# smritip/real-time-audio-sync

Measured on AMD Instinct MI355X. Metric: aligned chroma frames/sec, batch=64 OTW c=500; path-index match vs CPU ref, higher is better.
Workload: dtype f64 arithmetic, f32 features in HBM

## Files before the change

### real_time_audio_sync_amd/csrc/otw.hip

```cpp
#include <hip/hip_runtime.h>
#include <math.h>
#include <stddef.h>
#include <stdint.h>
#include <stdlib.h>
#include <string.h>
#include <type_traits>

#include "common.h"

namespace rts {

constexpr int kF = 12;
constexpr int kFetch = 8;

struct OtwArgs {
    const void *ref;
    const void *live;
    const int32_t *live_len;
    int32_t *state;
    int32_t *path;
    double *bands;
    long long live_stride;
    int N, c, max_run_count, variant, cost_kind, mode;
    int path_cap, live_cap;
    int ref_f64, live_f64;
    int clamp_len;
    long long *debug;
    int spec;
    double *dense_acc;
    double *dense_cost;
    const long long *ref_first;
    const int32_t *ref_len;
};

struct LiveFromGlobal {};
struct LiveFromGlobalLean {};
template <typename RT> struct RingElem { using type = RT; };
template <> struct RingElem<LiveFromGlobal> { using type = float; };
template <> struct RingElem<LiveFromGlobalLean> { using type = float; };
template <typename RT> constexpr bool kThroughput = std::is_same<RT, LiveFromGlobalLean>::value;
template <typename RT> constexpr bool kHasLiveRing = !std::is_same<RT, LiveFromGlobal>::value && !kThroughput<RT>;

template <int W, typename RT>
struct OtwLds {
    static constexpr int L = W / 64;
    static constexpr int SWZ = L * 65;
    double R[SWZ];
    double C[SWZ];
    double Dr[2][SWZ];
    double Dc[2][SWZ];
    using E = typename RingElem<RT>::type;
    E livew[kF][kHasLiveRing<RT> ? W : 1];
    double cfresh_min;
    double corner_pa;
    double corner_d;
    int cfresh_idx;
    int rfresh_idx;
    double rfresh_min;
    int plan_t[2], plan_j0[2], plan_flags[2];
    int t, j;
    E refw[kF][W];
};

struct OtwSpecOut {
    double min;
    double d;
    double d2;
    int idx;
    int flag;
};
template <int W>
struct alignas(16) OtwSpecLds {
    static constexpr int SWZ = (W / 64) * 65;
    double ShR[SWZ];
    double ShC[SWZ];
    OtwSpecOut row[2], col[2];
};

template <int W>
__device__ __forceinline__ int swz(int k) {
    constexpr int L = W / 64;
    const int p = k & (W - 1);
    return (p % L) * 65 + (p / L);
}

__device__ __forceinline__ double dmin(double a, double b) { return (b < a) ? b : a; }

__device__ __forceinline__ double dot_strided12(const double (&x)[kF], const double (&y)[kF]) {
    double t1 = 0.0, t2 = 0.0;
#pragma unroll
    for (int i = 0; i < kF; i += 4) {
        const double m3 = y[i + 2] * x[i + 2];
        const double m4 = y[i + 3] * x[i + 3];
        const double a = fma(y[i], x[i], m3);
        const double b = fma(y[i + 1], x[i + 1], m4);
        t1 = t1 + a;
        t2 = t2 + b;
    }
    return t1 + t2;
}

__device__ __forceinline__ double euclid12(const double (&a)[kF], const double (&b)[kF]) {
    double sq[kF];
#pragma unroll
    for (int i = 0; i < kF; i++) {
        const double d = a[i] - b[i];
        sq[i] = d * d;
    }
    double res = ((sq[0] + sq[1]) + (sq[2] + sq[3])) + ((sq[4] + sq[5]) + (sq[6] + sq[7]));
    res = res + sq[8];
    res = res + sq[9];
    res = res + sq[10];
    res = res + sq[11];
    return sqrt(res);
}

__device__ __forceinline__ double cell_cost(const double (&lf)[kF], const double (&rf)[kF], int euclid) {
    return euclid ? euclid12(lf, rf) : (1.0 - dot_strided12(lf, rf));
}

__device__ __forceinline__ double vmin(double a, double b) {
    double r;
    asm("v_min_f64 %0, %1, %2" : "=v"(r) : "v"(a), "v"(b));
    return r;
}

__device__ __forceinline__ double wave_shift_up(double v, double lane0) {
    const int lo = __builtin_amdgcn_update_dpp(__double2loint(lane0), __double2loint(v), 0x138, 0xf, 0xf, false);
    const int hi = __builtin_amdgcn_update_dpp(__double2hiint(lane0), __double2hiint(v), 0x138, 0xf, 0xf, false);
    return __hiloint2double(hi, lo);
}

__device__ __forceinline__ double wave_bcast(double v, int src_lane) {
    const int lo = __builtin_amdgcn_readlane(__double2loint(v), src_lane);
    const int hi = __builtin_amdgcn_readlane(__double2hiint(v), src_lane);
    return __hiloint2double(hi, lo);
}

__device__ __forceinline__ double rfl(double v) {
    const int lo = __builtin_amdgcn_readfirstlane(__double2loint(v));
    const int hi = __builtin_amdgcn_readfirstlane(__double2hiint(v));
    return __hiloint2double(hi, lo);
}

#define RTS_DPP_MIN_STEP(CTRL, ROWMASK)                                                                       \
    do {                                                                                                      \
        const int tlo = __builtin_amdgcn_update_dpp(__double2loint(x), __double2loint(x), CTRL, ROWMASK, 0xf, false); \
        const int thi = __builtin_amdgcn_update_dpp(__double2hiint(x), __double2hiint(x), CTRL, ROWMASK, 0xf, false); \
        x = vmin(x, __hiloint2double(thi, tlo));                                                              \
    } while (0)

__device__ __forceinline__ double wave_min(double x) {
    RTS_DPP_MIN_STEP(0x111, 0xf);
    RTS_DPP_MIN_STEP(0x112, 0xf);
    RTS_DPP_MIN_STEP(0x114, 0xf);
    RTS_DPP_MIN_STEP(0x118, 0xf);
    RTS_DPP_MIN_STEP(0x142, 0xa);
    RTS_DPP_MIN_STEP(0x143, 0xc);
    return wave_bcast(x, 63);
}

__device__ __forceinline__ unsigned lds_addr(const double *p) {
    return (unsigned)(uintptr_t)(__attribute__((address_space(3))) const double *)p;
}
template <int OFF>
__device__ __forceinline__ double lds_read_imm(unsigned addr) {
    double r;
    asm volatile("ds_read_b64 %0, %1 offset:%2" : "=v"(r) : "v"(addr), "n"(OFF));
    return r;
}
template <int OFF>
__device__ __forceinline__ void lds_write_imm(unsigned addr, double v) {
    asm volatile("ds_write_b64 %0, %1 offset:%2" ::"v"(addr), "v"(v), "n"(OFF) : "memory");
}
template <int L, int R, int M = 0>
__device__ __forceinline__ void chain_load(unsigned bA, unsigned bB, unsigned dA, unsigned dB, double (&prevb)[L + 1],
                                           double (&D)[L]) {
    if constexpr (M <= L) {
        constexpr int off = ((R + M) & (L - 1)) * 65 * 8;
        constexpr bool wrap = (R + M) >= L;
        prevb[M] = lds_read_imm<off>(wrap ? bB : bA);
        if constexpr (M > 0) D[M - 1] = lds_read_imm<off>(wrap ? dB : dA);
        chain_load<L, R, M + 1>(bA, bB, dA, dB, prevb, D);
    }
}
template <int L, int M = 0>
__device__ __forceinline__ void chain_wait(double (&prevb)[L + 1], double (&D)[L]) {
    if constexpr (M == 0) asm volatile("s_waitcnt lgkmcnt(0)" ::: "memory");
    if constexpr (M <= L) {
        asm volatile("" : "+v"(prevb[M]));
        if constexpr (M < L) asm volatile("" : "+v"(D[M]));
        chain_wait<L, M + 1>(prevb, D);
    }
}
template <int L, int R, int M = 1>
__device__ __forceinline__ void chain_store(unsigned oA, unsigned oB, const double (&v)[L], double v_top) {
    if constexpr (M <= L) {
        constexpr int off = ((R + M) & (L - 1)) * 65 * 8;
        lds_write_imm<off>((R + M) >= L ? oB : oA, (M == L) ? v_top : v[M - 1]);
        chain_store<L, R, M + 1>(oA, oB, v, v_top);
    }
}

template <int W, bool DENSE, bool GUARD = false, bool ALT = false>
__device__ __forceinline__ void strip_chain(const double *__restrict__ Dv, const double *band, double *band_out, int k1,
                                            int n, double x_in, int lane, int lo_arg, double &fmin_out, int &fidx_out,
                                            double *dense_acc, double *dense_cost, long long dense_stride,
                                            long long *rounds_acc = nullptr, bool prev0_xin = false, double alt_xin = 0.0,
                                            int *alt_ok = nullptr) {
    constexpr int L = W / 64;
    constexpr int LOG_L = (L == 1) ? 0 : (L == 2) ? 1 : (L == 4) ? 2 : (L == 8) ? 3 : (L == 16) ? 4 : 5;
    const double inf = INFINITY;
    int slot[L + 1];
    const int nloc = n - L * lane;
    double prevb[L + 1], D[L], v[L];
    const int q0 = k1 - 1 + W;
    const int r0 = q0 & (L - 1);
    const int colA = ((q0 >> LOG_L) + lane) & 63, colB = (colA + 1) & 63;
    if constexpr (GUARD) {
        const unsigned bA = lds_addr(band + colA), bB = lds_addr(band + colB), dA = lds_addr(Dv + colA), dB = lds_addr(Dv + colB);
        switch (r0) {
#define RTS_CHAIN_LOAD(R)                                                        \
    case R:                                                                      \
        if constexpr (R < L) chain_load<L, R>(bA, bB, dA, dB, prevb, D);         \
        break;
            RTS_CHAIN_LOAD(0) RTS_CHAIN_LOAD(1) RTS_CHAIN_LOAD(2) RTS_CHAIN_LOAD(3) RTS_CHAIN_LOAD(4) RTS_CHAIN_LOAD(5)
            RTS_CHAIN_LOAD(6) RTS_CHAIN_LOAD(7) RTS_CHAIN_LOAD(8) RTS_CHAIN_LOAD(9) RTS_CHAIN_LOAD(10) RTS_CHAIN_LOAD(11)
            RTS_CHAIN_LOAD(12) RTS_CHAIN_LOAD(13) RTS_CHAIN_LOAD(14) RTS_CHAIN_LOAD(15)
            RTS_CHAIN_LOAD(16) RTS_CHAIN_LOAD(17) RTS_CHAIN_LOAD(18) RTS_CHAIN_LOAD(19) RTS_CHAIN_LOAD(20) RTS_CHAIN_LOAD(21)
            RTS_CHAIN_LOAD(22) RTS_CHAIN_LOAD(23) RTS_CHAIN_LOAD(24) RTS_CHAIN_LOAD(25) RTS_CHAIN_LOAD(26) RTS_CHAIN_LOAD(27)
            RTS_CHAIN_LOAD(28) RTS_CHAIN_LOAD(29) RTS_CHAIN_LOAD(30) RTS_CHAIN_LOAD(31)
#undef RTS_CHAIN_LOAD
        }
        chain_wait<L>(prevb, D);
    } else {
#pragma unroll
        for (int m = 0; m <= L; m++) {
            const int q = k1 + m - 1 + W;
            slot[m] = (q & (L - 1)) * 65 + (((q >> LOG_L) + lane) & 63);
        }
#pragma unroll
        for (int m = 0; m <= L; m++) prevb[m] = band[slot[m]];
#pragma unroll
        for (int m = 0; m < L; m++) D[m] = Dv[slot[m + 1]];
    }
    prevb[0] = (k1 == 0 && lane == 0) ? inf : prevb[0];
    if (GUARD && ALT) prevb[0] = (prev0_xin && lane == 0) ? x_in : prevb[0];
#pragma unroll
    for (int m = 0; m < L; m++) D[m] = (m < nloc) ? D[m] : inf;
    double p = (lane == 0) ? x_in : inf;
    double am1 = inf;
#pragma unroll
    for (int m = 0; m < L; m++) {
        const double am = vmin(prevb[m + 1] + D[m], prevb[m] + 2 * D[m]);
        if (GUARD && ALT && m == 1) am1 = am;
        p = p + D[m];
        v[m] = vmin(am, p);
        p = v[m];
    }
    if (GUARD && ALT && L >= 2) {
        if (alt_ok) *alt_ok = __builtin_amdgcn_readfirstlane((int)(vmin(am1, alt_xin + D[1]) == v[1]));
    }
    for (int round = 0; round < 64; round++) {
        double q = wave_shift_up(v[L - 1], x_in);
        q = q + D[0];
        if (!__any(q < v[0])) break;
        if (rounds_acc) *rounds_acc += 1;
        v[0] = vmin(v[0], q);
#pragma unroll
        for (int m = 1; m < L; m++) {
            q = q + D[m];
            v[m] = vmin(v[m], q);
        }
    }
    if constexpr (GUARD) {
        const double v_top = (lane == 63) ? x_in : v[L - 1];
        const unsigned oA = lds_addr(band_out + colA), oB = lds_addr(band_out + colB);
        switch (r0) {
#define RTS_CHAIN_STORE(R)                                                       \
    case R:                                                                      \
        if constexpr (R < L) chain_store<L, R>(oA, oB, v, v_top);                \
        break;
            RTS_CHAIN_STORE(0) RTS_CHAIN_STORE(1) RTS_CHAIN_STORE(2) RTS_CHAIN_STORE(3) RTS_CHAIN_STORE(4)
            RTS_CHAIN_STORE(5) RTS_CHAIN_STORE(6) RTS_CHAIN_STORE(7) RTS_CHAIN_STORE(8) RTS_CHAIN_STORE(9)
            RTS_CHAIN_STORE(10) RTS_CHAIN_STORE(11) RTS_CHAIN_STORE(12) RTS_CHAIN_STORE(13) RTS_CHAIN_STORE(14)
            RTS_CHAIN_STORE(15) RTS_CHAIN_STORE(16) RTS_CHAIN_STORE(17) RTS_CHAIN_STORE(18) RTS_CHAIN_STORE(19)
            RTS_CHAIN_STORE(20) RTS_CHAIN_STORE(21) RTS_CHAIN_STORE(22) RTS_CHAIN_STORE(23) RTS_CHAIN_STORE(24)
            RTS_CHAIN_STORE(25) RTS_CHAIN_STORE(26) RTS_CHAIN_STORE(27) RTS_CHAIN_STORE(28) RTS_CHAIN_STORE(29)
            RTS_CHAIN_STORE(30) RTS_CHAIN_STORE(31)
#undef RTS_CHAIN_STORE
        }
    } else {
#pragma unroll
        for (int m = 0; m < L; m++) band_out[slot[m + 1]] = v[m];
    }
    if (DENSE) {
#pragma unroll
        for (int m = 0; m < L; m++) {
            if (m < nloc) {
                const long long off = (long long)(L * lane + m) * dense_stride;
                dense_acc[off] = v[m];
                dense_cost[off] = D[m];
            }
        }
    }
    const double v0 = (lane == 0 && lo_arg > k1) ? inf : v[0];
    double lm = v0;
#pragma unroll
    for (int m = 1; m < L; m++) lm = vmin(lm, v[m]);
    const double g = wave_min(lm);
    int ml = L;
#pragma unroll
    for (int m = L - 1; m >= 1; m--) ml = (v[m] == g) ? m : ml;
    ml = (v0 == g) ? 0 : ml;
    const unsigned long long mask = __ballot(ml != L);
    const bool some = (g < inf) && (mask != 0);
    const int first = (int)__builtin_ctzll(mask | (1ull << 63));
    fmin_out = g;
    fidx_out = some ? k1 + L * first + __builtin_amdgcn_readlane(ml, first) : 0x7fffffff;
}

template <int W>
__device__ __forceinline__ void band_argmin(const double *__restrict__ band, int lo, int hi, int lane,
                                            double &vmin_out, int &imin) {
    constexpr int L = W / 64;
    double v[L];
    double lm = INFINITY;
#pragma unroll
    for (int m = 0; m < L; m++) {
        const int k = lo + L * lane + m;
        v[m] = (k <= hi) ? band[swz<W>(k)] : (double)INFINITY;
        if (k <= hi) lm = vmin(lm, v[m]);
    }
    const double g = wave_min(lm);
    int cand = 0x7fffffff;
#pragma unroll
    for (int m = L - 1; m >= 0; m--) {
        const int k = lo + L * lane + m;
        if (k <= hi && v[m] == g) cand = k;
    }
    const unsigned long long mask = __ballot(cand != 0x7fffffff);
    vmin_out = g;
    imin = mask ? __builtin_amdgcn_readlane(cand, (int)__builtin_ctzll(mask)) : 0x7fffffff;
}

#if defined(RTS_OTW_STAMPS) && RTS_OTW_STAMPS == 1
#define RTS_STAMP2(slot)      \
    do {                      \
        if (stamp_base)       \
            RTS_STAMP(8 + slot); \
        else                  \
            RTS_STAMP(slot);  \
    } while (0)
#define RTS_STAMP(slot)                                                   \
    do {                                                                  \
        const long long now_ = (long long)__builtin_amdgcn_s_memtime();   \
        __builtin_amdgcn_s_waitcnt(0xC07F);                               \
        stamp_sum[slot] += now_ - stamp_last;                             \
        stamp_last = now_;                                                \
    } while (0)
#else
#define RTS_STAMP(slot) \
    do {                \
    } while (0)
#define RTS_STAMP2(slot) \
    do {                 \
    } while (0)
#endif

struct OtwCtl {
    int t, j, dir, prev, run_count, status, first, n_path, consumed, rows, cols, truncated, pend_dir;
    int recomputes, pending_col, last_x, last_y, rb_idx, cb_idx;
    int live_hi, ref_hi;
    int spec_valid;
    int ri, ci;
    double cA, cU, cL;
    long long cells;
    double rb_min, cb_min;
    double pfl0, pfl1, pfr0, pfr1;
};

struct OtwEnv {
    int b, lane, c, N, live_len, live_cap, euclid, variant, mode, max_run_count, path_cap, live_f64, ref_f64;
    long long live_base;
    const void *live, *ref;
    int32_t *path;
    bool deferred_update;
};

constexpr int kPlanRow = 1, kPlanCol = 2, kPlanStop = 4, kPlanExit = 8;
constexpr int kPlanHit = 16;
constexpr int kPlanRi = 32, kPlanCi = 64;
// ... 466 lines not shown
        otw_ref_frame(e, kb_c, rb);
        const double da = cell_cost(lf, ra, e.euclid), db = cell_cost(lf, rb, e.euclid);
        Drow[swz<W>(ka)] = da;
        if (ka >= dual_lo) S.Dc[ka & 1][swz<W>(r)] = da;
        if (kb <= k_hi) {
            Drow[swz<W>(kb)] = db;
            if (kb >= dual_lo) S.Dc[kb & 1][swz<W>(r)] = db;
        }
    }
}
template <int W, typename RT>
__device__ __forceinline__ void otw_cost_col(OtwLds<W, RT> &S, const OtwEnv &e, int q, int r_lo, int r_hi, int dual_lo,
                                             int hidx, int hn) {
    if (q >= e.N) return;
    const int lim = (e.live_len < e.live_cap) ? e.live_len : e.live_cap;
    if (r_lo < 0) r_lo = 0;
    if (r_hi > lim - 1) r_hi = lim - 1;
    if (r_lo + hidx > r_hi) return;
    double *Dcol = S.Dc[q & 1];
    double rf[kF];
    otw_ref_frame(e, q, rf);
    if constexpr (kThroughput<RT>) {
        for (int ra_ = r_lo + hidx; ra_ <= r_hi; ra_ += hn) {
            double la[kF];
            otw_live_frame(e, ra_, la);
            const double da = cell_cost(la, rf, e.euclid);
            Dcol[swz<W>(ra_)] = da;
            if (ra_ >= dual_lo) S.Dr[ra_ & 1][swz<W>(q)] = da;
        }
        return;
    }
    for (int ra_ = r_lo + hidx; ra_ <= r_hi; ra_ += 2 * hn) {
        const int rb_ = ra_ + hn;
        const int rb_c = (rb_ <= r_hi) ? rb_ : ra_;
        double la[kF], lb[kF];
        if constexpr (!kHasLiveRing<RT>) {
            otw_live_frame(e, ra_, la);
            otw_live_frame(e, rb_c, lb);
        } else {
#pragma unroll
            for (int f = 0; f < kF; f++) {
                la[f] = (double)S.livew[f][ra_ & (W - 1)];
                lb[f] = (double)S.livew[f][rb_c & (W - 1)];
            }
        }
        const double da = cell_cost(la, rf, e.euclid), db = cell_cost(lb, rf, e.euclid);
        Dcol[swz<W>(ra_)] = da;
        if (ra_ >= dual_lo) S.Dr[ra_ & 1][swz<W>(q)] = da;
        if (rb_ <= r_hi) {
            Dcol[swz<W>(rb_)] = db;
            if (rb_ >= dual_lo) S.Dr[rb_ & 1][swz<W>(q)] = db;
        }
    }
}

template <int W, typename RT>
__device__ __forceinline__ void otw_costs_prime(OtwLds<W, RT> &S, const OtwEnv &e, int t, int j, int hidx, int hn) {
    const int c = e.c;
    const int none = 0x7fffffff;
    otw_cost_row<W, RT>(S, e, t + 1, j - c + 1, j + 2, none, hidx, hn);
    otw_cost_row<W, RT>(S, e, t + 2, j - c + 1, j + 2, none, hidx, hn);
    otw_cost_col<W, RT>(S, e, j + 1, t - c + 1, t + 2, none, hidx, hn);
    otw_cost_col<W, RT>(S, e, j + 2, t - c + 1, t + 2, none, hidx, hn);
}

template <int W, typename RT>
__device__ __forceinline__ void otw_costs_advance(OtwLds<W, RT> &S, const OtwEnv &e, int pt, int jn, bool do_row,
                                                  bool do_col, int hidx, int hn) {
    const int c = e.c;
    if (do_row) otw_cost_row<W, RT>(S, e, pt + 2, jn - c + 1, jn + 2, jn + 1, hidx, hn);
    if (do_col) otw_cost_col<W, RT>(S, e, jn + 2, pt - c + 1, pt + 2, pt + 1, hidx, hn);
}

template <int W, bool ALT>
__device__ __forceinline__ void otw_spec_strip(const double *Dv, const double *band, double *shadow, int pos, int c,
                                               int lane, double sentinel, OtwSpecOut *out, long long *rounds_acc = nullptr,
                                               bool prev0_sentinel = false) {
    const int k1 = (pos - c + 1 > 0) ? pos - c + 1 : 0;
    double fm;
    int fi;
    const double d_last = Dv[swz<W>(pos)];
    const double d_next = Dv[swz<W>(pos + 1)];
    int alt_ok = 0;
    strip_chain<W, false, true, ALT>(Dv, band, shadow, k1, pos - k1, (k1 > 0) ? sentinel : (double)INFINITY, lane, k1, fm, fi,
                                nullptr, nullptr, 0, rounds_acc, prev0_sentinel, sentinel, &alt_ok);
    if (lane == 0) {
        out->min = fm;
        out->idx = fi;
        out->d = d_last;
        out->d2 = d_next;
        out->flag = alt_ok;
    }
}

__device__ __forceinline__ double otw_last_cell_from(double prev_raw, int pos, int k1, double side_v, double diag_v, double d,
                                                     double sentinel) {
    const double inf = INFINITY;
    const int n = pos - k1;
    const double prev = (n > 0) ? prev_raw : ((k1 > 0) ? sentinel : inf);
    const double diag = (pos > 0) ? diag_v + 2 * d : inf;
    return vmin(vmin(side_v + d, diag), prev + d);
}
template <int W>
__device__ __forceinline__ double otw_last_cell(const double *band, int pos, int k1, double side_v, double diag_v, double d,
                                                double sentinel) {
    const int n = pos - k1;
    return otw_last_cell_from(band[swz<W>(pos - (n > 0 ? 1 : 0))], pos, k1, side_v, diag_v, d, sentinel);
}

template <int W, typename RT>
__device__ __forceinline__ OtwSettled otw_settle_hit_both(double *R, double *C, const OtwSpecOut *exr, const OtwSpecOut *exc,
                                                          OtwCtl &k, const OtwEnv &e, int pt, int j0, double sentinel) {
    const int c = e.c, lane = e.lane;
    const int jn = j0 + 1, t0 = pt - 1;
    if (e.deferred_update && k.pend_dir != -2) {
        k.run_count = (k.pend_dir == k.prev) ? k.run_count + 1 : 1;
        if (k.pend_dir != RTS_DIR_BOTH) k.prev = k.pend_dir;
        k.pend_dir = -2;
    }
    const int k1r_ = (j0 - c + 1 > 0) ? j0 - c + 1 : 0, k1c_ = (pt - c + 1 > 0) ? pt - c + 1 : 0;
    const double pra_raw = R[swz<W>(j0 - (j0 - k1r_ > 0 ? 1 : 0))], prb_raw = C[swz<W>(t0 - (t0 - k1c_ > 0 ? 1 : 0))];
    const double d1_raw = exr->d, d2_raw = exc->d, d3_raw = exc->d2, rmin_raw = exr->min, cmin_raw = exc->min;
    const int ridx_raw = exr->idx, cidx_raw = exc->idx;
    const double d1 = rfl(d1_raw), d2 = rfl(d2_raw), d3 = rfl(d3_raw);
    double rmin = rfl(rmin_raw), cmin = rfl(cmin_raw);
    int ridx = __builtin_amdgcn_readfirstlane(ridx_raw), cidx = __builtin_amdgcn_readfirstlane(cidx_raw);
    const double pra = rfl(pra_raw), prb = rfl(prb_raw);
    const int k1r = (j0 - c + 1 > 0) ? j0 - c + 1 : 0, k1c = (pt - c + 1 > 0) ? pt - c + 1 : 0;
    const int lo_r = (jn - c + 1 > 0) ? jn - c + 1 : 0;
    const int k1c_s = (t0 - c + 1 > 0) ? t0 - c + 1 : 0;
    const double a = rfl(otw_last_cell_from(pra, j0, k1r, k.cA, k.cL, d1, sentinel));
    const double b = rfl(otw_last_cell_from(prb, t0, k1c, k.cA, k.cU, d2, sentinel));
    const double pa = k.cA + 2 * d3;
    const double av = vmin(a + d3, pa);
    const double cl = vmin(av, b + d3);
    if (lane == 0) {
        R[swz<W>(j0)] = a;
        C[swz<W>(t0)] = b;
        R[swz<W>(jn)] = cl;
        C[swz<W>(pt)] = cl;
        if (k1c > k1c_s) C[swz<W>(k1c - 1)] = sentinel;
    }
    if (a < rmin) {
        rmin = a;
        ridx = j0;
    }
    if (b < cmin) {
        cmin = b;
        cidx = t0;
    }
    const bool row_ok = ridx >= lo_r, col_ok = cidx >= k1c;
    if (!row_ok) k.rb_idx = -1;
    if (!col_ok) k.cb_idx = -1;
    k.rows += 1;
    k.cols += 1;
    k.consumed = pt + 1;
    k.cells += (j0 - k1r + 1) + (pt - k1c + 1);
    k.cU = b;
    k.cL = a;
    k.cA = cl;
    OtwSettled o;
    o.row_fresh = row_ok;
    o.col_fresh = col_ok;
    o.rf_min = rmin;
    o.rf_idx = ridx;
    o.cf_min = cmin;
    o.cf_idx = cidx;
    o.row_corner = o.col_corner = true;
    o.rc = o.cc = cl;
    o.stop = false;
    return o;
}

__device__ __forceinline__ int otw_resolve_plan(int pflags, int pt, int c, const OtwSpecOut *exc) {
    if (pflags & kPlanHitIf) {
        const bool ok = (pt < c) || __builtin_amdgcn_readfirstlane(exc->flag) != 0;
        if (ok) pflags = (pflags | kPlanHit) ^ (kPlanRi | kPlanCi);
    }
    return pflags;
}

template <int W, typename RT>
__device__ __forceinline__ OtwSettled otw_settle_hit(double *R, double *C, const OtwSpecOut *ex, OtwCtl &k, const OtwEnv &e,
                                                     int pt, int j0, bool is_row, double sentinel) {
    const int c = e.c, lane = e.lane;
    const double inf = INFINITY;
    const int jn = j0 + (is_row ? 0 : 1);
    const int pos = is_row ? j0 : pt;
    const int k1 = (pos - c + 1 > 0) ? pos - c + 1 : 0;
    const int n = pos - k1;
    double *band = is_row ? R : C;
    double *other = is_row ? C : R;
    if (e.deferred_update && k.pend_dir != -2) {
        k.run_count = (k.pend_dir == k.prev) ? k.run_count + 1 : 1;
        if (k.pend_dir != RTS_DIR_BOTH) k.prev = k.pend_dir;
        k.pend_dir = -2;
    }
    const double prev_raw = band[swz<W>(pos - (n > 0 ? 1 : 0))];
    const double d_raw = ex->d, smin_raw = ex->min;
    const int sidx_raw = ex->idx;
    const double d = rfl(d_raw);
    const double smin = rfl(smin_raw);
    const int sidx = __builtin_amdgcn_readfirstlane(sidx_raw);
    const double prev_s = rfl(prev_raw);
    const double prev = (n > 0) ? prev_s : ((k1 > 0) ? sentinel : inf);
    const double side = k.cA + d;
    const double diag = (pos > 0) ? (is_row ? k.cL : k.cU) + 2 * d : inf;
    const double cl = vmin(vmin(side, diag), prev + d);
    if (lane == 0) {
        band[swz<W>(pos)] = cl;
        other[swz<W>(is_row ? pt : jn)] = cl;
    }
    if (is_row) {
        k.rows += 1;
        k.consumed = pt + 1;
        k.cU = k.cA;
        k.cL = prev;
    } else {
        k.cols += 1;
        k.cL = k.cA;
        k.cU = prev;
    }
    k.cA = cl;
    k.cells += n + 1;
    OtwSettled o;
    o.row_fresh = is_row;
    o.col_fresh = !is_row;
    o.rf_min = o.cf_min = smin;
    o.rf_idx = o.cf_idx = sidx;
    o.row_corner = o.col_corner = true;
    o.rc = o.cc = cl;
    o.stop = false;
    return o;
}

#ifdef RTS_OTW_FULL_BARRIER
#define RTS_STEP_BARRIER() __syncthreads()
#else
#define RTS_STEP_BARRIER() ::rts::lds_barrier()
#endif

template <int W, int NW, bool DENSE, typename RT, bool SPEC>
__global__ void __launch_bounds__(64 * NW) __attribute__((amdgpu_waves_per_eu(kThroughput<RT> ? 6 : 1)))
otw_advance_kernel(OtwArgs a) {
    static_assert(!SPEC || (NW >= 8 && !DENSE), "the pipelined kernel needs 8 waves and no dense mirror");
    constexpr int NT = 64 * NW;
    constexpr int HW0 = SPEC ? 3 : (NW >= 4) ? 2 : 0;
    constexpr int NHELP = 64 * (NW - HW0);
#if defined(RTS_OTW_STAMPS) && RTS_OTW_STAMPS == 1
    long long stamp_sum[16] = {0, 0, 0, 0, 0, 0, 0, 0, 0, 0, 0, 0, 0, 0, 0, 0};
    int stamp_base = 0;
    long long stamp_last = (long long)__builtin_amdgcn_s_memtime();
    __builtin_amdgcn_s_waitcnt(0xC07F);
#endif
#if defined(RTS_OTW_STAMPS) && RTS_OTW_STAMPS == 2
    long long lw_hit = 0, lb_hit = 0, lw_oth = 0, lb_oth = 0, ln_hit = 0, ln_oth = 0, l_last = 0;
    long long lo_work = 0, lo_t0 = 0;
    long long lo_rounds = 0;
#define RTS_ROUNDS_ACC (&lo_rounds)
#define RTS_LW_BEGIN() do { lo_t0 = (long long)__builtin_amdgcn_s_memtime(); __builtin_amdgcn_s_waitcnt(0xC07F); } while (0)
#define RTS_LW_END(hit) do { const long long t_ = (long long)__builtin_amdgcn_s_memtime(); __builtin_amdgcn_s_waitcnt(0xC07F); if (hit) lo_work += t_ - lo_t0; } while (0)
#else
#define RTS_ROUNDS_ACC nullptr
#define RTS_LW_BEGIN() do { } while (0)
#define RTS_LW_END(hit) do { } while (0)
#endif
    extern __shared__ __align__(16) unsigned char smem_raw[];
    OtwLds<W, RT> &S = *reinterpret_cast<OtwLds<W, RT> *>(smem_raw);
    using LdsT = OtwLds<W, RT>;
    constexpr bool kNoLiveRing = !kHasLiveRing<RT>;
    constexpr bool kRefRing = !SPEC && !kNoLiveRing;
    constexpr size_t kSpecOff = (offsetof(LdsT, refw) + 15) & ~(size_t)15;
    OtwSpecLds<W> &SP = *reinterpret_cast<OtwSpecLds<W> *>(smem_raw + kSpecOff);

    const int tid = threadIdx.x;
    const int lane = tid & 63;
    const int wave = __builtin_amdgcn_readfirstlane(tid >> 6);
    const double sentinel = (a.variant == RTS_VARIANT_OTW) ? 1e10 : (double)INFINITY;
    const double inf = INFINITY;
    OtwEnv e;
    e.b = blockIdx.x;
    e.lane = lane;
    e.c = a.c;
    e.euclid = a.cost_kind == RTS_COST_EUCLID;
    e.variant = a.variant;
    e.mode = a.mode;
// ... 189 lines not shown
                const int pt = __builtin_amdgcn_readfirstlane(S.plan_t[sp]), j0 = __builtin_amdgcn_readfirstlane(S.plan_j0[sp]);
                const int pflags = otw_resolve_plan(__builtin_amdgcn_readfirstlane(S.plan_flags[sp]), pt, c, &SP.col[sp]);
                if (pflags & kPlanExit) break;
                const bool do_row = (pflags & kPlanRow) != 0, do_col = (pflags & kPlanCol) != 0;
                RTS_LW_BEGIN();
                if constexpr (!kNoLiveRing)
                    if (wave == HW0) otw_refill<W, RT>(S, k, e, pt + 3, 0, false);
                if (!(pflags & kPlanHit)) RTS_STEP_BARRIER();
                if (!(pflags & kPlanStop))
                    otw_costs_advance<W, RT>(S, e, pt, j0 + (do_col ? 1 : 0), do_row, do_col, tid - 64 * HW0, NHELP);
                RTS_LW_END(pflags & kPlanHit);
                RTS_STEP_BARRIER();
                sp ^= 1;
            }
        } else if (wave == 1) {
            for (;;) {
                const int pt = __builtin_amdgcn_readfirstlane(S.plan_t[sp]), j0 = __builtin_amdgcn_readfirstlane(S.plan_j0[sp]);
                const int pflags = otw_resolve_plan(__builtin_amdgcn_readfirstlane(S.plan_flags[sp]), pt, c, &SP.col[sp]);
                if (pflags & kPlanExit) break;
                const int jn = j0 + ((pflags & kPlanCol) ? 1 : 0);
                double *R = (pflags & kPlanRi) ? SP.ShR : S.R, *Rsh = (pflags & kPlanRi) ? S.R : SP.ShR;
                RTS_LW_BEGIN();
                if (!(pflags & kPlanHit)) {
                    if ((pflags & (kPlanRow | kPlanCol | kPlanStop)) == (kPlanRow | kPlanCol))
                        otw_col_strip<W, DENSE, RT>(S, (pflags & kPlanCi) ? SP.ShC : S.C, a, e, S.Dc[(j0 + 1) & 1], pt,
                                                    j0 + 1, true, sentinel);
                    RTS_STEP_BARRIER();
                }
                if ((pflags & (kPlanHit | kPlanRow | kPlanCol)) == (kPlanHit | kPlanRow | kPlanCol)) {
                    const double av = otw_last_cell<W>(R, j0, (j0 - c + 1 > 0) ? j0 - c + 1 : 0, Rsh[swz<W>(j0)],
                                                       Rsh[swz<W>(j0 > 0 ? j0 - 1 : 0)], SP.row[sp].d, sentinel);
                    if (lane == 0) R[swz<W>(j0)] = av;
                }
                if (!(pflags & kPlanStop) && pt + 1 < live_len && pt + 1 < e.live_cap)
                    otw_spec_strip<W, false>(S.Dr[(pt + 1) & 1], R, Rsh, jn, c, lane, sentinel, &SP.row[sp ^ 1], RTS_ROUNDS_ACC);
                RTS_LW_END(pflags & kPlanHit);
                RTS_STEP_BARRIER();
                sp ^= 1;
            }
        } else if (wave == 2) {
            for (;;) {
                const int pt = __builtin_amdgcn_readfirstlane(S.plan_t[sp]), j0 = __builtin_amdgcn_readfirstlane(S.plan_j0[sp]);
                const int pflags = otw_resolve_plan(__builtin_amdgcn_readfirstlane(S.plan_flags[sp]), pt, c, &SP.col[sp]);
                if (pflags & kPlanExit) break;
                const int jn = j0 + ((pflags & kPlanCol) ? 1 : 0);
                double *C = (pflags & kPlanCi) ? SP.ShC : S.C, *Csh = (pflags & kPlanCi) ? S.C : SP.ShC;
                RTS_LW_BEGIN();
                if (!(pflags & kPlanHit)) {
                    if constexpr (kThroughput<RT>) {
                        const bool stop2 = (pflags & kPlanStop) != 0;
                        if (pflags & kPlanRow) {
                            double rf_min = inf;
                            int rf_idx = 0x7fffffff;
                            otw_row_strip<W, DENSE, RT>((pflags & kPlanRi) ? SP.ShR : S.R, a, e, S.Dr[pt & 1], pt, j0, jn, sentinel,
                                                        rf_min, rf_idx);
                            if (lane == 0) {
                                S.rfresh_min = rf_min;
                                S.rfresh_idx = rf_idx;
                            }
                        } else if ((pflags & kPlanCol) && !stop2) {
                            otw_col_strip<W, DENSE, RT>(S, C, a, e, S.Dc[jn & 1], pt, jn, false, sentinel);
                        }
                    }
                    RTS_STEP_BARRIER();
                }
                bool drop = false;
                if ((pflags & (kPlanHit | kPlanRow | kPlanCol)) == (kPlanHit | kPlanRow | kPlanCol)) {
                    const int t0 = pt - 1;
                    const double bv = otw_last_cell<W>(C, t0, (pt - c + 1 > 0) ? pt - c + 1 : 0, Csh[swz<W>(t0)],
                                                       Csh[swz<W>(t0 > 0 ? t0 - 1 : 0)], SP.col[sp].d, sentinel);
                    if (lane == 0) C[swz<W>(t0)] = bv;
                    drop = pt >= c;
                }
                if (!(pflags & kPlanStop) && jn + 1 < N)
                    otw_spec_strip<W, true>(S.Dc[(jn + 1) & 1], C, Csh, pt, c, lane, sentinel, &SP.col[sp ^ 1], RTS_ROUNDS_ACC, drop);
                RTS_LW_END(pflags & kPlanHit);
                RTS_STEP_BARRIER();
                sp ^= 1;
            }
        } else {
#if defined(RTS_OTW_STAMPS) && RTS_OTW_STAMPS == 2
            l_last = (long long)__builtin_amdgcn_s_memtime();
            __builtin_amdgcn_s_waitcnt(0xC07F);
#endif
            for (;;) {
                RTS_STAMP2(0);
                const int pt = __builtin_amdgcn_readfirstlane(pl.t), j0 = __builtin_amdgcn_readfirstlane(pl.j0);
                pl.flags = __builtin_amdgcn_readfirstlane(pl.flags);
                const int pflags = otw_resolve_plan(pl.flags, pt, c, &SP.col[sp]);
                if (pflags & kPlanExit) break;
                if ((pl.flags & kPlanHitIf) && (pflags & kPlanHit)) {
                    k.ri ^= 1;
                    k.ci ^= 1;
                }
                const bool do_row = (pflags & kPlanRow) != 0, do_col = (pflags & kPlanCol) != 0;
                const bool stop = (pflags & kPlanStop) != 0;
                const int jn = j0 + (do_col ? 1 : 0);
                double *R = (pflags & kPlanRi) ? SP.ShR : S.R, *C = (pflags & kPlanCi) ? SP.ShC : S.C;
                OtwSettled o;
#if defined(RTS_OTW_STAMPS) && RTS_OTW_STAMPS == 1
                stamp_base = (pflags & kPlanHit) ? 0 : 8;
                if (stamp_base) stamp_sum[14] += 1; else stamp_sum[6] += 1;
#endif
                if (pflags & kPlanHit) RTS_STAMP(1);
                if ((pflags & kPlanHit) && do_row && do_col) {
                    o = otw_settle_hit_both<W, RT>(R, C, &SP.row[sp], &SP.col[sp], k, e, pt, j0, sentinel);
                } else if (pflags & kPlanHit) {
                    o = otw_settle_hit<W, RT>(R, C, do_row ? &SP.row[sp] : &SP.col[sp], k, e, pt, j0, do_row, sentinel);
                } else {
                    double rf_min = inf;
                    int rf_idx = 0x7fffffff;
                    if constexpr (!kThroughput<RT>) {
                        if (do_row)
                            otw_row_strip<W, DENSE, RT>(R, a, e, S.Dr[pt & 1], pt, j0, jn, sentinel, rf_min, rf_idx);
                        else if (do_col && !stop)
                            otw_col_strip<W, DENSE, RT>(S, C, a, e, S.Dc[jn & 1], pt, jn, false, sentinel);
                    }
                    RTS_STAMP(9);
                    RTS_STEP_BARRIER();
                    RTS_STAMP(10);
                    if constexpr (kThroughput<RT>) {
                        if (do_row) {
                            rf_min = rfl(S.rfresh_min);
                            rf_idx = __builtin_amdgcn_readfirstlane(S.rfresh_idx);
                        }
                    }
                    const double ld_u = C[swz<W>(pt > 0 ? pt - 1 : 0)], ld_l = R[swz<W>(jn > 0 ? jn - 1 : 0)];
                    o = otw_settle<W, DENSE, RT>(S, R, C, k, a, e, pt, j0, pflags, rf_min, rf_idx, sentinel);
                    k.cA = o.cc;
                    k.cU = (pt > 0) ? rfl(ld_u) : inf;
                    k.cL = (jn > 0) ? rfl(ld_l) : inf;
                }
                RTS_STAMP2(3);
                if (o.stop) {
                    k.status = RTS_STOP_REF_END;
                    k.t = pt;
                    k.j = jn;
                    k.pending_col = 0;
                } else {
                    otw_decide<W, RT>(R, C, k, e, pt, jn, o.row_fresh, o.rf_min, o.rf_idx, o.col_fresh, o.cf_min, o.cf_idx,
                                      o.row_corner, o.rc, o.col_corner, o.cc, false);
                }
                RTS_STAMP2(4);
                k.spec_valid = !o.stop;
                pl = otw_make_plan<W, RT>(S, k, e, true, sp ^ 1);
                RTS_STAMP2(5);
#if defined(RTS_OTW_STAMPS) && RTS_OTW_STAMPS == 2
                {
                    const long long t0_ = (long long)__builtin_amdgcn_s_memtime();
                    __builtin_amdgcn_s_waitcnt(0xC07F);
                    RTS_STEP_BARRIER();
                    const long long t1_ = (long long)__builtin_amdgcn_s_memtime();
                    __builtin_amdgcn_s_waitcnt(0xC07F);
                    if (pflags & kPlanHit) {
                        lw_hit += t0_ - l_last;
                        lb_hit += t1_ - t0_;
                        ln_hit += 1;
                    } else {
                        lw_oth += t0_ - l_last;
                        lb_oth += t1_ - t0_;
                        ln_oth += 1;
                    }
                    l_last = t1_;
                }
#else
                RTS_STEP_BARRIER();
#endif
                sp ^= 1;
            }
        }
    } else if constexpr (NW >= 4) {
        if (wave >= HW0) {
            for (;;) {
                const int pt = __builtin_amdgcn_readfirstlane(S.plan_t[0]), j0 = __builtin_amdgcn_readfirstlane(S.plan_j0[0]),
                          pflags = __builtin_amdgcn_readfirstlane(S.plan_flags[0]);
                if (pflags & kPlanExit) break;
                const int jn = j0 + ((pflags & kPlanCol) ? 1 : 0);
                if (!(pflags & kPlanStop))
                    otw_precompute<W, RT>(S, e, pt, jn, S.Dr[buf ^ 1], S.Dc[buf ^ 1], tid - 64 * HW0, NHELP);
                __syncthreads();
                __syncthreads();
                buf ^= 1;
            }
        } else if (wave == 1) {
            for (;;) {
                const int pt = __builtin_amdgcn_readfirstlane(S.plan_t[0]), j0 = __builtin_amdgcn_readfirstlane(S.plan_j0[0]),
                          pflags = __builtin_amdgcn_readfirstlane(S.plan_flags[0]);
                if (pflags & kPlanExit) break;
                if ((pflags & (kPlanRow | kPlanCol | kPlanStop)) == (kPlanRow | kPlanCol))
                    otw_col_strip<W, DENSE, RT>(S, S.C, a, e, S.Dc[buf], pt, j0 + 1, true, sentinel);
                __syncthreads();
                __syncthreads();
                buf ^= 1;
            }
        } else {
            for (;;) {
                RTS_STAMP(0);
                const int pt = __builtin_amdgcn_readfirstlane(S.plan_t[0]), j0 = __builtin_amdgcn_readfirstlane(S.plan_j0[0]),
                          pflags = __builtin_amdgcn_readfirstlane(S.plan_flags[0]);
                if (pflags & kPlanExit) break;
                const bool do_row = (pflags & kPlanRow) != 0, do_col = (pflags & kPlanCol) != 0;
                const bool stop = (pflags & kPlanStop) != 0;
                const int jn = j0 + (do_col ? 1 : 0);
                double rf_min = inf;
                int rf_idx = 0x7fffffff;
                if (do_row)
                    otw_row_strip<W, DENSE, RT>(S.R, a, e, S.Dr[buf], pt, j0, jn, sentinel, rf_min, rf_idx);
                else if (do_col && !stop)
                    otw_col_strip<W, DENSE, RT>(S, S.C, a, e, S.Dc[buf], pt, jn, false, sentinel);
                RTS_STAMP(3);
                __syncthreads();
                RTS_STAMP(5);
                const OtwSettled o = otw_settle<W, DENSE, RT>(S, S.R, S.C, k, a, e, pt, j0, pflags, rf_min, rf_idx, sentinel);
                otw_finish<W, RT>(S, k, e, pt, jn, o);
                RTS_STAMP(8);
                __syncthreads();
                buf ^= 1;
            }
        }
    } else {
        for (;;) {
            RTS_STAMP(0);
            const int pt = __builtin_amdgcn_readfirstlane(S.plan_t[0]), j0 = __builtin_amdgcn_readfirstlane(S.plan_j0[0]),
                      pflags = __builtin_amdgcn_readfirstlane(S.plan_flags[0]);
            if (pflags & kPlanExit) break;
            const bool do_row = (pflags & kPlanRow) != 0, do_col = (pflags & kPlanCol) != 0;
            const bool stop = (pflags & kPlanStop) != 0;
            const int jn = j0 + (do_col ? 1 : 0);
            const int k1r = (j0 - c + 1 > 0) ? j0 - c + 1 : 0, nr = j0 - k1r + 1;
            const int k1c = (pt - c + 1 > 0) ? pt - c + 1 : 0, nc = pt - k1c + 1;
            const bool col_active = do_col && !stop;
            double *Dr = S.Dr[buf], *Dc = S.Dc[buf];

            const int col_wave = (NW > 1 && do_row) ? 1 : 0;
            double rf_min = inf;
            int rf_idx = 0x7fffffff;
            if (do_row && wave == 0) {
                const double x_in = (k1r > 0) ? sentinel : inf;
                const int lo_arg = (jn - c + 1 > 0) ? jn - c + 1 : 0;
                const long long dro = ((long long)e.b * e.live_cap + pt) * N + k1r;
                strip_chain<W, DENSE>(Dr, S.R, S.R, k1r, nr, x_in, lane, lo_arg, rf_min, rf_idx, DENSE ? a.dense_acc + dro : nullptr,
                                      DENSE ? a.dense_cost + dro : nullptr, 1);
                if (lane == 0 && k1r > 0) S.R[swz<W>(k1r - 1)] = sentinel;
            }
            if (col_active && wave == col_wave) {
                const double x_in = (k1c > 0) ? sentinel : inf;
                const int ncc = nc - (do_row ? 1 : 0);
                double fm;
                int fi;
                const double dcorner = Dc[swz<W>(pt)];
                const double pa = (do_row && pt > 0) ? S.C[swz<W>(pt - 1)] + 2 * dcorner : inf;
                const long long dco = ((long long)e.b * e.live_cap + k1c) * N + jn;
// ... 686 lines not shown
```

Before: 32.34 million.

## Defer speculative strip argmin reduction to consumer and add fast hit-step loop

The speculative strip worker now writes per-lane partial minima and indices to LDS, and skips the wave-wide min and ballot. The consuming wave does that reduction itself, which shortens the speculative worker's critical path. A specialized inner loop handles consecutive row- or column-hit plan steps for W=512 latency mode, with templated variant and defer flags and uniform control state. In exchange, the consumer does extra reduction work and reads more from LDS, and the code grows.

Result: faster. 33.16 million, median of 6 (+2.5%).

```diff
diff --git a/real_time_audio_sync_amd/csrc/otw.hip b/real_time_audio_sync_amd/csrc/otw.hip
--- a/real_time_audio_sync_amd/csrc/otw.hip
+++ b/real_time_audio_sync_amd/csrc/otw.hip
@@ -63,10 +63,11 @@
 };
 
 struct OtwSpecOut {
-    double min;
+    double pmin[64];
+    int pidx[64];
     double d;
     double d2;
-    int idx;
+    int k1;
     int flag;
 };
 template <int W>
@@ -202,7 +203,7 @@
     }
 }
 
-template <int W, bool DENSE, bool GUARD = false, bool ALT = false>
+template <int W, bool DENSE, bool GUARD = false, bool ALT = false, bool SPLIT = false>
 __device__ __forceinline__ void strip_chain(const double *__restrict__ Dv, const double *band, double *band_out, int k1,
                                             int n, double x_in, int lane, int lo_arg, double &fmin_out, int &fidx_out,
                                             double *dense_acc, double *dense_cost, long long dense_stride,
@@ -308,6 +309,15 @@
     double lm = v0;
 #pragma unroll
     for (int m = 1; m < L; m++) lm = vmin(lm, v[m]);
+    if constexpr (SPLIT) {
+        int mfirst = L;
+#pragma unroll
+        for (int m = L - 1; m >= 1; m--) mfirst = (v[m] == lm) ? m : mfirst;
+        mfirst = (v0 == lm) ? 0 : mfirst;
+        fmin_out = lm;
+        fidx_out = mfirst;
+        return;
+    }
     const double g = wave_min(lm);
     int ml = L;
 #pragma unroll
@@ -940,15 +950,27 @@
     const double d_last = Dv[swz<W>(pos)];
     const double d_next = Dv[swz<W>(pos + 1)];
     int alt_ok = 0;
-    strip_chain<W, false, true, ALT>(Dv, band, shadow, k1, pos - k1, (k1 > 0) ? sentinel : (double)INFINITY, lane, k1, fm, fi,
-                                nullptr, nullptr, 0, rounds_acc, prev0_sentinel, sentinel, &alt_ok);
+    strip_chain<W, false, true, ALT, true>(Dv, band, shadow, k1, pos - k1, (k1 > 0) ? sentinel : (double)INFINITY, lane, k1,
+                                           fm, fi, nullptr, nullptr, 0, rounds_acc, prev0_sentinel, sentinel, &alt_ok);
+    out->pmin[lane] = fm;
+    out->pidx[lane] = fi;
     if (lane == 0) {
-        out->min = fm;
-        out->idx = fi;
+        out->k1 = k1;
         out->d = d_last;
         out->d2 = d_next;
         out->flag = alt_ok;
     }
+}
+
+template <int W>
+__device__ __forceinline__ void otw_spec_argmin(double lm, int ml, int k1, double &g_out, int &idx_out) {
+    constexpr int L = W / 64;
+    const double g = wave_min(lm);
+    const unsigned long long mask = __ballot(lm == g);
+    const bool some = (g < INFINITY) && (mask != 0);
+    const int first = (int)__builtin_ctzll(mask | (1ull << 63));
+    g_out = g;
+    idx_out = some ? k1 + L * first + __builtin_amdgcn_readlane(ml, first) : 0x7fffffff;
 }
 
 __device__ __forceinline__ double otw_last_cell_from(double prev_raw, int pos, int k1, double side_v, double diag_v, double d,
@@ -978,11 +1000,15 @@
     }
     const int k1r_ = (j0 - c + 1 > 0) ? j0 - c + 1 : 0, k1c_ = (pt - c + 1 > 0) ? pt - c + 1 : 0;
     const double pra_raw = R[swz<W>(j0 - (j0 - k1r_ > 0 ? 1 : 0))], prb_raw = C[swz<W>(t0 - (t0 - k1c_ > 0 ? 1 : 0))];
-    const double d1_raw = exr->d, d2_raw = exc->d, d3_raw = exc->d2, rmin_raw = exr->min, cmin_raw = exc->min;
-    const int ridx_raw = exr->idx, cidx_raw = exc->idx;
+    const double d1_raw = exr->d, d2_raw = exc->d, d3_raw = exc->d2, rlm = exr->pmin[lane], clm = exc->pmin[lane];
+    const int rml = exr->pidx[lane], cml = exc->pidx[lane], rk1 = exr->k1, ck1 = exc->k1;
     const double d1 = rfl(d1_raw), d2 = rfl(d2_raw), d3 = rfl(d3_raw);
-    double rmin = rfl(rmin_raw), cmin = rfl(cmin_raw);
-    int ridx = __builtin_amdgcn_readfirstlane(ridx_raw), cidx = __builtin_amdgcn_readfirstlane(cidx_raw);
+    double rmin, cmin;
+    int ridx, cidx;
+    otw_spec_argmin<W>(rlm, rml, __builtin_amdgcn_readfirstlane(rk1), rmin, ridx);
+    otw_spec_argmin<W>(clm, cml, __builtin_amdgcn_readfirstlane(ck1), cmin, cidx);
+    rmin = rfl(rmin), cmin = rfl(cmin);
+    ridx = __builtin_amdgcn_readfirstlane(ridx), cidx = __builtin_amdgcn_readfirstlane(cidx);
     const double pra = rfl(pra_raw), prb = rfl(prb_raw);
     const int k1r = (j0 - c + 1 > 0) ? j0 - c + 1 : 0, k1c = (pt - c + 1 > 0) ? pt - c + 1 : 0;
     const int lo_r = (jn - c + 1 > 0) ? jn - c + 1 : 0;
@@ -1055,11 +1081,14 @@
         k.pend_dir = -2;
     }
     const double prev_raw = band[swz<W>(pos - (n > 0 ? 1 : 0))];
-    const double d_raw = ex->d, smin_raw = ex->min;
-    const int sidx_raw = ex->idx;
+    const double d_raw = ex->d, lm = ex->pmin[lane];
+    const int ml = ex->pidx[lane], sk1 = ex->k1;
     const double d = rfl(d_raw);
-    const double smin = rfl(smin_raw);
-    const int sidx = __builtin_amdgcn_readfirstlane(sidx_raw);
+    double smin_v;
+    int sidx_v;
+    otw_spec_argmin<W>(lm, ml, __builtin_amdgcn_readfirstlane(sk1), smin_v, sidx_v);
+    const double smin = rfl(smin_v);
+    const int sidx = __builtin_amdgcn_readfirstlane(sidx_v);
     const double prev_s = rfl(prev_raw);
     const double prev = (n > 0) ? prev_s : ((k1 > 0) ? sentinel : inf);
     const double side = k.cA + d;
@@ -1415,8 +1444,157 @@
 #if defined(RTS_OTW_STAMPS) && RTS_OTW_STAMPS == 2
             l_last = (long long)__builtin_amdgcn_s_memtime();
             __builtin_amdgcn_s_waitcnt(0xC07F);
+#define RTS_W0_STEP_END(hit)                                              \
+    do {                                                                  \
+        const long long t0_ = (long long)__builtin_amdgcn_s_memtime();    \
+        __builtin_amdgcn_s_waitcnt(0xC07F);                               \
+        RTS_STEP_BARRIER();                                               \
+        const long long t1_ = (long long)__builtin_amdgcn_s_memtime();    \
+        __builtin_amdgcn_s_waitcnt(0xC07F);                               \
+        if (hit) {                                                        \
+            lw_hit += t0_ - l_last;                                       \
+            lb_hit += t1_ - t0_;                                          \
+            ln_hit += 1;                                                  \
+        } else {                                                          \
+            lw_oth += t0_ - l_last;                                       \
+            lb_oth += t1_ - t0_;                                          \
+            ln_oth += 1;                                                  \
+        }                                                                 \
+        l_last = t1_;                                                     \
+    } while (0)
+#else
+#define RTS_W0_STEP_END(hit) RTS_STEP_BARRIER()
 #endif
+            int2 *const path_row = reinterpret_cast<int2 *>(e.path) + (size_t)e.b * e.path_cap;
+            const auto hit_steps = [&](auto v2_c, auto defer_c) __attribute__((always_inline)) {
+                constexpr bool V2 = decltype(v2_c)::value, DEFER = decltype(defer_c)::value;
+#define RTS_RFL_CTL(f) k.f = __builtin_amdgcn_readfirstlane(k.f)
+                RTS_RFL_CTL(t), RTS_RFL_CTL(j), RTS_RFL_CTL(dir), RTS_RFL_CTL(prev), RTS_RFL_CTL(run_count);
+                RTS_RFL_CTL(status), RTS_RFL_CTL(n_path), RTS_RFL_CTL(consumed), RTS_RFL_CTL(rows), RTS_RFL_CTL(cols);
+                RTS_RFL_CTL(truncated), RTS_RFL_CTL(pend_dir), RTS_RFL_CTL(pending_col), RTS_RFL_CTL(last_x);
+                RTS_RFL_CTL(last_y), RTS_RFL_CTL(spec_valid), RTS_RFL_CTL(ri), RTS_RFL_CTL(ci);
+#undef RTS_RFL_CTL
+                for (;;) {
+                    const int pt = __builtin_amdgcn_readfirstlane(pl.t), j0 = __builtin_amdgcn_readfirstlane(pl.j0);
+                    const int fl = __builtin_amdgcn_readfirstlane(pl.flags);
+                    const int kind = fl & (kPlanHit | kPlanRow | kPlanCol | kPlanStop | kPlanExit | kPlanHitIf);
+                    const bool is_row = kind == (kPlanHit | kPlanRow);
+                    if (!is_row && kind != (kPlanHit | kPlanCol)) return;
+                    const int jn = is_row ? j0 : j0 + 1;
+                    const int keep_lo = is_row ? pt - c + 1 : jn - c + 1;
+                    const int keep_idx = __builtin_amdgcn_readfirstlane(is_row ? k.cb_idx : k.rb_idx);
+                    if (keep_idx < ((keep_lo > 0) ? keep_lo : 0)) return;
+#if defined(RTS_OTW_STAMPS) && RTS_OTW_STAMPS == 1
+                    stamp_base = 0;
+                    stamp_sum[6] += 1;
+#endif
+                    RTS_STAMP(0);
+                    RTS_STAMP(1);
+                    double *R = (fl & kPlanRi) ? SP.ShR : S.R, *C = (fl & kPlanCi) ? SP.ShC : S.C;
+                    const int pos = is_row ? j0 : pt;
+                    const int k1 = (pos - c + 1 > 0) ? pos - c + 1 : 0;
+                    const int n = pos - k1;
+                    double *band = is_row ? R : C, *other = is_row ? C : R;
+                    const OtwSpecOut *ex = is_row ? &SP.row[sp] : &SP.col[sp];
+                    if constexpr (DEFER) {
+                        if (k.pend_dir != -2) {
+                            k.run_count = (k.pend_dir == k.prev) ? k.run_count + 1 : 1;
+                            if (k.pend_dir != RTS_DIR_BOTH) k.prev = k.pend_dir;
+                            k.pend_dir = -2;
+                        }
+                    }
+                    const double prev_raw = band[swz<W>(pos - (n > 0 ? 1 : 0))];
+                    const double d = ex->d, lm = ex->pmin[lane];
+                    const int ml = ex->pidx[lane], sk1 = ex->k1;
+                    double smin;
+                    int sidx;
+                    otw_spec_argmin<W>(lm, ml, __builtin_amdgcn_readfirstlane(sk1), smin, sidx);
+                    const double prev = (n > 0) ? prev_raw : ((k1 > 0) ? sentinel : inf);
+                    const double diag = (pos > 0) ? (is_row ? k.cL : k.cU) + 2 * d : inf;
+                    const double cl = vmin(vmin(k.cA + d, diag), prev + d);
+                    if (lane == 0) {
+                        band[swz<W>(pos)] = cl;
+                        other[swz<W>(is_row ? pt : jn)] = cl;
+                    }
+                    if (is_row) {
+                        k.rows += 1;
+                        k.consumed = pt + 1;
+                        k.cU = k.cA;
+                        k.cL = prev;
+                    } else {
+                        k.cols += 1;
+                        k.cL = k.cA;
+                        k.cU = prev;
+                    }
+                    k.cA = cl;
+                    k.cells += n + 1;
+                    RTS_STAMP(3);
+                    double rmin = is_row ? smin : k.rb_min, cmin = is_row ? k.cb_min : smin;
+                    int ridx = is_row ? sidx : k.rb_idx, cidx = is_row ? k.cb_idx : sidx;
+                    const bool r_new = cl < rmin, c_new = cl < cmin;
+                    rmin = r_new ? cl : rmin;
+                    ridx = r_new ? jn : ridx;
+                    cmin = c_new ? cl : cmin;
+                    cidx = c_new ? pt : cidx;
+                    k.rb_min = rmin;
+                    k.rb_idx = ridx;
+                    k.cb_min = cmin;
+                    k.cb_idx = cidx;
+                    const bool rlt = rmin < cmin;
+                    const int x = rlt ? pt : cidx, y = rlt ? ridx : jn;
+                    bool append = true;
+                    if constexpr (V2) {
+                        const int xs = __builtin_amdgcn_readfirstlane(x), ys = __builtin_amdgcn_readfirstlane(y);
+                        append = (k.n_path == 0) || (xs > k.last_x && ys >= k.last_y);
+                        if (append) {
+                            k.last_x = xs;
+                            k.last_y = ys;
+                        }
+                    }
+                    if (append) {
+                        if (k.n_path < e.path_cap) {
+                            if (lane == 0) path_row[k.n_path] = make_int2(x, y);
+                        } else {
+                            k.truncated = 1;
+                        }
+                        k.n_path += 1;
+                    }
+                    int nd = __builtin_amdgcn_readfirstlane((x < pt) ? RTS_DIR_COLUMN : (y < jn) ? RTS_DIR_ROW : RTS_DIR_BOTH);
+                    if (pt < c)
+                        nd = RTS_DIR_BOTH;
+                    else if (k.run_count >= e.max_run_count)
+                        nd = (k.prev == RTS_DIR_ROW) ? RTS_DIR_COLUMN : RTS_DIR_ROW;
+                    if constexpr (DEFER) {
+                        k.pend_dir = nd;
+                    } else {
+                        k.run_count = (nd == k.prev) ? k.run_count + 1 : 1;
+                        if (nd != RTS_DIR_BOTH) k.prev = nd;
+                    }
+                    k.dir = nd;
+                    k.pending_col = (nd == RTS_DIR_COLUMN);
+                    k.t = pt;
+                    k.j = jn;
+                    RTS_STAMP(4);
+                    k.spec_valid = 1;
+                    pl = otw_make_plan<W, RT>(S, k, e, true, sp ^ 1);
+                    RTS_STAMP(5);
+                    RTS_W0_STEP_END(true);
+                    sp ^= 1;
+                }
+            };
             for (;;) {
+                if constexpr (W == 512 && !kThroughput<RT>) {
+                    if (e.variant == RTS_VARIANT_LIVENOTE_V2) {
+                        if (e.deferred_update)
+                            hit_steps(std::true_type{}, std::true_type{});
+                        else
+                            hit_steps(std::true_type{}, std::false_type{});
+                    } else if (e.deferred_update) {
+                        hit_steps(std::false_type{}, std::true_type{});
+                    } else {
+                        hit_steps(std::false_type{}, std::false_type{});
+                    }
+                }
                 RTS_STAMP2(0);
                 const int pt = __builtin_amdgcn_readfirstlane(pl.t), j0 = __builtin_amdgcn_readfirstlane(pl.j0);
                 pl.flags = __builtin_amdgcn_readfirstlane(pl.flags);
@@ -1478,29 +1656,10 @@
                 k.spec_valid = !o.stop;
                 pl = otw_make_plan<W, RT>(S, k, e, true, sp ^ 1);
                 RTS_STAMP2(5);
-#if defined(RTS_OTW_STAMPS) && RTS_OTW_STAMPS == 2
-                {
-                    const long long t0_ = (long long)__builtin_amdgcn_s_memtime();
-                    __builtin_amdgcn_s_waitcnt(0xC07F);
-                    RTS_STEP_BARRIER();
-                    const long long t1_ = (long long)__builtin_amdgcn_s_memtime();
-                    __builtin_amdgcn_s_waitcnt(0xC07F);
-                    if (pflags & kPlanHit) {
-                        lw_hit += t0_ - l_last;
-                        lb_hit += t1_ - t0_;
-                        ln_hit += 1;
-                    } else {
-                        lw_oth += t0_ - l_last;
-                        lb_oth += t1_ - t0_;
-                        ln_oth += 1;
-                    }
-                    l_last = t1_;
-                }
-#else
-                RTS_STEP_BARRIER();
-#endif
+                RTS_W0_STEP_END(pflags & kPlanHit);
                 sp ^= 1;
             }
+#undef RTS_W0_STEP_END
         }
     } else if constexpr (NW >= 4) {
         if (wave >= HW0) {
```
